# fusioninfer/fusioninfer

Hardware: AMD Instinct MI355X
Metric: goodput req/s (Qwen3-8B serving, closed-loop) (higher is better)
Workload: dtype bf16; 1 GPU; model=Qwen3-8B, global_batch=256, seq_len=1152, prompt_len=1024, gen_len=128, parallelism=dp1

## Files before the change

fusioninfer_amd/ops/__init__.py:

```python

from __future__ import annotations

import math
from typing import Optional

import torch

from fusioninfer_amd.ops import reference as ref

_C = None
_C_IMPORT_ERROR: Optional[BaseException] = None
try:
    import importlib

    _C = importlib.import_module("fusioninfer_amd.ops._C")
except Exception as e:
    _C_IMPORT_ERROR = e


def has_native() -> bool:
    return _C is not None


def _require_native():
# ... 148 lines not shown
        if (k_cache.dim() != 4 or k_cache.shape != v_cache.shape
                or k_cache.shape[1] != num_kv_heads or k_cache.shape[2] != 16
                or k_cache.shape[3] != head_dim):
            raise ValueError(
                "rope_qk_norm_cache_: caches must both be "
                f"[B, {num_kv_heads}, 16, {head_dim}], got "
                f"{tuple(k_cache.shape)} and {tuple(v_cache.shape)}")
        _C.rope_qk_norm_cache(
            q, k, v, q_weight, k_weight, cos_sin, positions, k_cache,
            v_cache, slot_mapping, num_q_heads, num_kv_heads, head_dim, eps,
            k_inv_scale, v_inv_scale,
        )
        return q
    rope_qk_norm_(q, k, positions, cos_sin, num_q_heads, num_kv_heads,
                  head_dim, q_weight, k_weight, eps)
    reshape_and_cache(k, v, k_cache, v_cache, slot_mapping,
                      k_inv_scale, v_inv_scale)
    return q


def gather_kv_blocks(k_cache, v_cache, block_ids) -> torch.Tensor:
    if k_cache.is_cuda:
        _require_native()
        n = int(block_ids.numel())
        staging = torch.empty(
            (2, n, *k_cache.shape[1:]), dtype=k_cache.dtype, device=k_cache.device
        )
        _C.gather_kv_blocks(staging, k_cache, v_cache, block_ids)
        return staging
    return ref.gather_kv_blocks(k_cache, v_cache, block_ids.long())


def scatter_kv_blocks(staging, k_cache, v_cache, block_ids):
    if k_cache.is_cuda:
        _require_native()
        _C.scatter_kv_blocks(staging, k_cache, v_cache, block_ids)
        return
    ref.scatter_kv_blocks(staging, k_cache, v_cache, block_ids.long())



DECODE_PARTITION_TOKENS = 512


def _check_attn_out(out: torch.Tensor, q: torch.Tensor) -> None:
    if (out.shape != q.shape or out.dtype != q.dtype
            or out.device != q.device or not out.is_contiguous()):
        raise ValueError(
            f"out must be a contiguous {tuple(q.shape)} {q.dtype} tensor on "
            f"{q.device}, got {tuple(out.shape)} {out.dtype} strides "
            f"{out.stride()} on {out.device}")


def paged_attention_decode(
    q: torch.Tensor,
    k_cache: torch.Tensor,
    v_cache: torch.Tensor,
    block_tables: torch.Tensor,
    seq_lens: torch.Tensor,
    scale: Optional[float] = None,
    out: Optional[torch.Tensor] = None,
) -> torch.Tensor:
    if scale is None:
        scale = 1.0 / math.sqrt(q.shape[-1])
    if out is not None:
        _check_attn_out(out, q)
    if q.is_cuda:
        _require_native()
        S, Hq, D = q.shape
        if out is None:
            out = torch.empty(q.shape, dtype=q.dtype, device=q.device)
        max_tokens = int(block_tables.shape[1]) * int(k_cache.shape[2])
        num_parts = max(
            (max_tokens + DECODE_PARTITION_TOKENS - 1) // DECODE_PARTITION_TOKENS,
            1,
        )
        ml_ws = acc_ws = None
        if num_parts > 1:
            ml_ws = torch.empty(
                (S, Hq, num_parts, 2), dtype=torch.float32, device=q.device
            )
            acc_ws = torch.empty(
                (S, Hq, num_parts, D), dtype=torch.float32, device=q.device
            )
        _C.paged_attention_decode(
            out, q, k_cache, v_cache, block_tables, seq_lens,
            ml_ws, acc_ws, num_parts, scale,
        )
        return out
    res = ref.paged_attention_decode(q, k_cache, v_cache, block_tables, seq_lens, scale)
    return res if out is None else out.copy_(res)


import os as _os

PREFILL_TILE_ROWS = (4 if _os.environ.get("FI_PF_NW", "8").startswith("4")
                     else 8) * 32


def prefill_tile_rows(seq_lens) -> int:
    if seq_lens and max(seq_lens) >= 4096:
        return 128
    return PREFILL_TILE_ROWS


def build_prefill_tiles(seq_lens, device=None, rows=None):
    rows = rows or PREFILL_TILE_ROWS
    tile_seq, tile_row0 = [], []
    for s, L in enumerate(seq_lens):
        for r0 in range(0, L, rows):
            tile_seq.append(s)
            tile_row0.append(r0)
    return (
        torch.tensor(tile_seq, dtype=torch.int32, device=device),
        torch.tensor(tile_row0, dtype=torch.int32, device=device),
    )


def prefill_attention(
    q: torch.Tensor,
    k: torch.Tensor,
    v: torch.Tensor,
    cu_seqlens: torch.Tensor,
    scale: Optional[float] = None,
    tile_seq: Optional[torch.Tensor] = None,
    tile_row0: Optional[torch.Tensor] = None,
    tile_rows: Optional[int] = None,
) -> torch.Tensor:
    if scale is None:
        scale = 1.0 / math.sqrt(q.shape[-1])
    if q.is_cuda:
        _require_native()
        if tile_seq is None:
            lens = (cu_seqlens[1:] - cu_seqlens[:-1]).tolist()
            tile_rows = tile_rows or prefill_tile_rows(lens)
            tile_seq, tile_row0 = build_prefill_tiles(
                lens, device=q.device, rows=tile_rows
            )
        out = torch.empty(q.shape, dtype=q.dtype, device=q.device)
        _C.prefill_attention(out, q, k, v, tile_seq, tile_row0, cu_seqlens,
# ... 274 lines not shown
```

fusioninfer_amd/ops/csrc/ops.hip:

```cpp

#include <torch/extension.h>

#include <c10/hip/HIPStream.h>
#include <hip/hip_runtime.h>

#include "common.h"

namespace fi {

template <bool FUSED_ADD, bool FP8_OUT>
void launch_rms_norm(void*, float*, const u16*, u16*, const u16*, float, int,
                     int, hipStream_t);
void launch_silu_and_mul(u16*, const u16*, int64_t, int, hipStream_t);
template <bool SILU_MUL>
void launch_row_quant_fp8(unsigned char*, float*, const u16*, int, int,
                          hipStream_t);
void launch_rope_qk_norm(u16*, u16*, int64_t, int64_t, const u16*, const u16*,
                         const float*, const int*, int, int, int, int, float,
                         hipStream_t);
void launch_reshape_and_cache(const u16*, const u16*, void*, void*,
                              const int*, int64_t, int64_t, int, int, int,
                              int, bool, float, float, hipStream_t);
void launch_rope_qk_norm_cache(u16*, const u16*, const u16*, int64_t, int64_t,
                               int64_t, const u16*, const u16*, const float*,
                               const int*, void*, void*, const int*, int, int,
                               int, int, float, bool, float, float,
                               hipStream_t);
template <bool GATHER>
void launch_kv_block_copy(u16*, u16*, u16*, const int*, int, int64_t,
                          hipStream_t);
void launch_paged_attn_decode(u16*, float*, float*, const u16*, const void*,
                              const void*, const int*, const int*, int,
                              int64_t, int, int, int, int, int, float, bool,
                              hipStream_t);
void launch_prefill_attn(u16*, const u16*, const void*, const void*,
                         const int*, const int*, const int*, const int*,
                         const int*, int, int, int64_t, int64_t, int64_t, int,
                         int, int, float, bool, int, hipStream_t);
void launch_moe_gemm(u16*, const u16*, const u16*, const int*, const int*,
                     const int*, int, int, int, int, bool, hipStream_t);
void launch_moe_gemm_fp8(u16*, const unsigned char*, const float*,
                         const unsigned char*, const float*, const int*,
                         const int*, const int*, int, int, int, int, bool,
                         hipStream_t);
void launch_moe_align(const int*, int*, int*, int*, int*, int, int, int,
                      int, int, int, hipStream_t);
void launch_moe_router_topk(const float*, float*, int*, int, int, int,
                            bool, hipStream_t);
void launch_moe_combine(u16*, const u16*, const int*, const float*, int, int,
                        int, hipStream_t);
void launch_lora_apply(u16*, u16*, const u16*, const int*, const u16*,
                       const u16*, const float*, int, int, int, int, int,
                       hipStream_t);
void launch_sample_tokens(int64_t*, const float*, const float*, const int*,
                          const float*, const float*, const int64_t*, int,
                          int, hipStream_t);
void launch_apply_penalties(float*, const int*, const int*, const float*, int,
                            int, int, hipStream_t);
void launch_penalty_counts_add(int*, const int*, const int64_t*, int, int,
                               int, hipStream_t);

}

namespace {

using fi::u16;

#define CHECK_BF16_CUDA(t)                                     \
  TORCH_CHECK((t).is_cuda(), #t " must be on GPU");            \
  TORCH_CHECK((t).scalar_type() == at::kBFloat16, #t " must be bf16")

u16* bf16_ptr(at::Tensor& t) { return reinterpret_cast<u16*>(t.data_ptr()); }
const u16* bf16_cptr(const at::Tensor& t) {
  return reinterpret_cast<const u16*>(t.data_ptr());
}

hipStream_t current_stream() {
  return c10::hip::getCurrentHIPStream().stream();
}

bool cache_is_fp8(const at::Tensor& t) {
  TORCH_CHECK(
      t.scalar_type() == at::kBFloat16 || t.scalar_type() == at::kFloat8_e4m3fn,
      "kv cache must be bf16 or float8_e4m3fn");
  return t.scalar_type() == at::kFloat8_e4m3fn;
}

// ... 183 lines not shown
    if (!w) return nullptr;
    CHECK_BF16_CUDA(*w);
    TORCH_CHECK(w->is_contiguous() && w->numel() == head_dim && aligned16(*w));
    return bf16_cptr(*w);
  };
  const u16* qw = weight_ptr(q_weight);
  const u16* kw = weight_ptr(k_weight);
  fi::launch_rope_qk_norm_cache(
      bf16_ptr(q), bf16_cptr(k), bf16_cptr(v), q.stride(0), k.stride(0),
      v.stride(0), qw, kw, cos_sin.data_ptr<float>(),
      positions.data_ptr<int>(), k_cache.data_ptr(), v_cache.data_ptr(),
      slot_mapping.data_ptr<int>(), static_cast<int>(tokens),
      static_cast<int>(num_q_heads), static_cast<int>(num_kv_heads),
      static_cast<int>(head_dim), static_cast<float>(eps), fp8,
      static_cast<float>(k_inv_scale), static_cast<float>(v_inv_scale),
      current_stream());
}

void gather_kv_blocks(at::Tensor staging, at::Tensor k_cache,
                      at::Tensor v_cache, at::Tensor block_ids) {
  TORCH_CHECK(staging.is_cuda() &&
              staging.scalar_type() == k_cache.scalar_type());
  TORCH_CHECK(block_ids.scalar_type() == at::kInt);
  const int n = block_ids.size(0);
  const int64_t block_elems = k_cache.size(1) * k_cache.size(2) *
      k_cache.size(3) * k_cache.element_size() / 2;
  fi::launch_kv_block_copy<true>(
      static_cast<fi::u16*>(staging.data_ptr()),
      static_cast<fi::u16*>(k_cache.data_ptr()),
      static_cast<fi::u16*>(v_cache.data_ptr()), block_ids.data_ptr<int>(), n,
      block_elems, current_stream());
}

void scatter_kv_blocks(at::Tensor staging, at::Tensor k_cache,
                       at::Tensor v_cache, at::Tensor block_ids) {
  TORCH_CHECK(staging.is_cuda() &&
              staging.scalar_type() == k_cache.scalar_type());
  TORCH_CHECK(block_ids.scalar_type() == at::kInt);
  const int n = block_ids.size(0);
  const int64_t block_elems = k_cache.size(1) * k_cache.size(2) *
      k_cache.size(3) * k_cache.element_size() / 2;
  fi::launch_kv_block_copy<false>(
      static_cast<fi::u16*>(staging.data_ptr()),
      static_cast<fi::u16*>(k_cache.data_ptr()),
      static_cast<fi::u16*>(v_cache.data_ptr()), block_ids.data_ptr<int>(), n,
      block_elems, current_stream());
}

void paged_attention_decode(at::Tensor out, at::Tensor q, at::Tensor k_cache,
                            at::Tensor v_cache, at::Tensor block_tables,
                            at::Tensor seq_lens,
                            c10::optional<at::Tensor> ml_ws,
                            c10::optional<at::Tensor> acc_ws,
                            int64_t num_parts, double scale) {
  CHECK_BF16_CUDA(out);
  CHECK_BF16_CUDA(q);
  const bool fp8 = cache_is_fp8(k_cache);
  TORCH_CHECK(block_tables.scalar_type() == at::kInt &&
              block_tables.is_contiguous());
  TORCH_CHECK(seq_lens.scalar_type() == at::kInt);
  TORCH_CHECK(q.dim() == 3);
  const int num_seqs = q.size(0);
  const int num_heads = q.size(1);
  const int head_dim = q.size(2);
  const int num_kv_heads = k_cache.size(1);
  TORCH_CHECK(k_cache.size(2) == 16, "cache block_size must be 16");
  TORCH_CHECK(q.stride(2) == 1 && q.stride(1) == head_dim);
  TORCH_CHECK(out.is_contiguous() && out.sizes() == q.sizes(),
              "out must be a contiguous [S, Hq, D] tensor");
  float* ml = nullptr;
  float* acc = nullptr;
  if (num_parts > 1) {
    TORCH_CHECK(ml_ws && acc_ws, "workspace required when num_parts > 1");
    ml = ml_ws->data_ptr<float>();
    acc = acc_ws->data_ptr<float>();
  }
  fi::launch_paged_attn_decode(
      bf16_ptr(out), ml, acc, bf16_cptr(q), k_cache.data_ptr(),
      v_cache.data_ptr(), block_tables.data_ptr<int>(),
      seq_lens.data_ptr<int>(), num_seqs, q.stride(0), block_tables.size(1),
      num_kv_heads, head_dim, num_heads / num_kv_heads,
      static_cast<int>(num_parts), static_cast<float>(scale), fp8,
      current_stream());
}

void prefill_attention(at::Tensor out, at::Tensor q, at::Tensor k,
                       at::Tensor v, at::Tensor tile_seq, at::Tensor tile_row0,
                       at::Tensor cu_seqlens, double scale,
                       int64_t tile_rows) {
  TORCH_CHECK(tile_rows == 128 || tile_rows == 256,
              "tile_rows must be 128 or 256");
  CHECK_BF16_CUDA(out);
  CHECK_BF16_CUDA(q);
  TORCH_CHECK(tile_seq.scalar_type() == at::kInt &&
              tile_row0.scalar_type() == at::kInt &&
              cu_seqlens.scalar_type() == at::kInt);
  TORCH_CHECK(q.dim() == 3 && k.dim() == 3 && v.dim() == 3);
  const int num_q_heads = q.size(1);
  const int head_dim = q.size(2);
  const int num_kv_heads = k.size(1);
  TORCH_CHECK(q.stride(2) == 1 && q.stride(1) == head_dim);
  TORCH_CHECK(k.stride(2) == 1 && k.stride(1) == head_dim);
  TORCH_CHECK(v.stride(2) == 1 && v.stride(1) == head_dim);
  fi::launch_prefill_attn(
      bf16_ptr(out), bf16_cptr(q), bf16_cptr(k), bf16_cptr(v),
      tile_seq.data_ptr<int>(), tile_row0.data_ptr<int>(),
      cu_seqlens.data_ptr<int>(), nullptr, nullptr, 0, tile_seq.size(0),
      q.stride(0), k.stride(0), v.stride(0), num_q_heads, num_kv_heads,
      head_dim, static_cast<float>(scale), false,
      static_cast<int>(tile_rows / 32), current_stream());
}

void prefill_attention_paged(at::Tensor out, at::Tensor q, at::Tensor k_cache,
                             at::Tensor v_cache, at::Tensor tile_seq,
                             at::Tensor tile_row0, at::Tensor cu_seqlens,
                             at::Tensor block_tables, at::Tensor seq_lens_k,
                             double scale, int64_t tile_rows) {
  TORCH_CHECK(tile_rows == 128 || tile_rows == 256,
              "tile_rows must be 128 or 256");
  CHECK_BF16_CUDA(out);
  CHECK_BF16_CUDA(q);
  const bool fp8 = cache_is_fp8(k_cache);
  TORCH_CHECK(tile_seq.scalar_type() == at::kInt &&
              tile_row0.scalar_type() == at::kInt &&
              cu_seqlens.scalar_type() == at::kInt &&
              block_tables.scalar_type() == at::kInt &&
              seq_lens_k.scalar_type() == at::kInt);
  TORCH_CHECK(block_tables.is_contiguous());
  TORCH_CHECK(q.dim() == 3);
  const int num_q_heads = q.size(1);
  const int head_dim = q.size(2);
  const int num_kv_heads = k_cache.size(1);
  TORCH_CHECK(k_cache.size(2) == 16, "cache block_size must be 16");
  TORCH_CHECK(q.stride(2) == 1 && q.stride(1) == head_dim);
  TORCH_CHECK(out.is_contiguous() && out.sizes() == q.sizes(),
              "out must be a contiguous [T, Hq, D] tensor");
// ... 227 lines not shown
      logits.data_ptr<float>(), counts.data_ptr<int>(),
      slot_ids.data_ptr<int>(), params.data_ptr<float>(),
      static_cast<int>(T), static_cast<int>(V),
      static_cast<int>(counts.size(0)), current_stream());
}

void penalty_counts_add(at::Tensor counts, at::Tensor slot_ids,
                        at::Tensor token_ids) {
  TORCH_CHECK(counts.is_cuda() && counts.scalar_type() == at::kInt &&
              counts.is_contiguous() && counts.dim() == 2 &&
              counts.size(0) >= 1 && counts.size(0) < (1LL << 31) &&
              counts.size(1) >= 1 && counts.size(1) < (1LL << 30),
              "penalty_counts_add: counts must be a contiguous [S >= 1, "
              "1 <= V < 2^30] int32 GPU tensor");
  const int64_t N = slot_ids.numel();
  TORCH_CHECK(N >= 1 && N < (1LL << 31) - 256,
              "penalty_counts_add: need 1 <= N < 2^31 - 256");
  TORCH_CHECK(slot_ids.is_cuda() && slot_ids.scalar_type() == at::kInt &&
              slot_ids.is_contiguous() && slot_ids.dim() == 1,
              "penalty_counts_add: bad slot_ids");
  TORCH_CHECK(token_ids.is_cuda() && token_ids.scalar_type() == at::kLong &&
              token_ids.is_contiguous() && token_ids.dim() == 1 &&
              token_ids.numel() == N,
              "penalty_counts_add: bad token_ids");
  fi::launch_penalty_counts_add(
      counts.data_ptr<int>(), slot_ids.data_ptr<int>(),
      token_ids.data_ptr<int64_t>(), static_cast<int>(N),
      static_cast<int>(counts.size(1)), static_cast<int>(counts.size(0)),
      current_stream());
}

}

PYBIND11_MODULE(TORCH_EXTENSION_NAME, m) {
  m.def("rms_norm", &rms_norm, "RMSNorm (bf16, fp32 accum)");
  m.def("fused_add_rms_norm", &fused_add_rms_norm,
        "in-place residual add + RMSNorm");
  m.def("silu_and_mul", &silu_and_mul, "fused SiLU-mul");
  m.def("rms_norm_fp8", &rms_norm_fp8, "RMSNorm with fused fp8 row quant");
  m.def("fused_add_rms_norm_fp8", &fused_add_rms_norm_fp8,
        "residual add + RMSNorm with fused fp8 row quant");
  m.def("silu_and_mul_fp8", &silu_and_mul_fp8,
        "fused SiLU-mul with fp8 row quant");
  m.def("quant_fp8_rows", &quant_fp8_rows, "per-row dynamic fp8 quant");
  m.def("rope_qk_norm", &rope_qk_norm,
        "fused per-head qk RMSNorm + NeoX RoPE (in-place)");
  m.def("reshape_and_cache", &reshape_and_cache, "scatter K/V into paged cache");
  m.def("rope_qk_norm_cache", &rope_qk_norm_cache,
        "fused qk RMSNorm + NeoX RoPE (q in place) + K/V paged-cache write");
  m.def("gather_kv_blocks", &gather_kv_blocks, "pack KV blocks for PD send");
  m.def("scatter_kv_blocks", &scatter_kv_blocks, "unpack KV blocks from PD recv");
  m.def("paged_attention_decode", &paged_attention_decode,
        "paged decode attention");
  m.def("prefill_attention", &prefill_attention, "varlen causal MFMA prefill");
  m.def("prefill_attention_paged", &prefill_attention_paged,
        "varlen causal MFMA prefill over the paged cache (context attention)");
  m.def("moe_gemm", &moe_gemm,
        "grouped MFMA GEMM over block-aligned expert segments "
        "(gate_up=true fuses the SwiGLU epilogue)");
  m.def("moe_gemm_fp8", &moe_gemm_fp8,
        "grouped fp8 (e4m3) MFMA GEMM with per-row/per-channel dequant "
        "epilogue (gate_up=true fuses SwiGLU)");
  m.def("moe_combine", &moe_combine,
        "weighted top-k combine of expert outputs (deterministic)");
  m.def("moe_align", &moe_align,
        "single-kernel block alignment of expert assignments "
        "(vLLM moe_align_block_size analog)");
  m.def("moe_router_topk", &moe_router_topk,
        "fused router tail: softmax + top-k + optional renormalize");
  m.def("lora_apply", &lora_apply,
        "batched multi-LoRA shrink + expand indexed by per-token slot ids "
        "(in-place on out)");
  m.def("sample_tokens", &sample_tokens,
        "fused temperature / top-k / top-p / min-p sampling with a "
        "counter-based (Philox4x32-10) draw, one workgroup per row");
  m.def("apply_penalties", &apply_penalties,
        "repetition / presence / frequency penalties from a per-slot token "
        "histogram (in-place on logits)");
  m.def("penalty_counts_add", &penalty_counts_add,
        "counts[slot_ids[i], token_ids[i]] += 1 (integer atomics)");
}
```

fusioninfer_amd/ops/csrc/paged_attention.hip:

```cpp

#include "common.h"

#include <type_traits>

namespace fi {

constexpr int kBlockSz = 16;
constexpr int kPartChunks = 32;
constexpr float kNegInf = -1e30f;
constexpr float kLog2e = 1.4426950408889634f;

typedef __attribute__((ext_vector_type(8))) short short8;
typedef __attribute__((ext_vector_type(4))) float floatx4;


template <typename CT_, int D, int G, int HS>
struct ScalarScores {
  using CT = CT_;
  static constexpr int G2 = G / HS, kTokLo = 4, kTokHi = 64;
  static constexpr int DPQ = D / 4;
  static constexpr int KQ4 = DPQ * sizeof(CT) / 16;
  static constexpr int EPG = 16 / sizeof(CT);
  struct KTile { uint4 v[KQ4]; };
  struct Q { const float (*heads)[D]; };

  static FI_DEV void init(Q& qs, const u16* q_row, float scale, int tid,
                          int nthreads, int, int hsplit) {
    __shared__ float q_lds[G][D];
    for (int e = tid; e < G * D; e += nthreads)
      q_lds[e / D][e % D] = bf16_to_f32(q_row[e]) * scale * kLog2e;
    __syncthreads();
    qs.heads = &q_lds[hsplit * G2];
  }

  static FI_DEV void load_k(const CT* k_block, int lane, KTile& k) {
    const CT* k_row = k_block + (lane / 4) * D + (lane % 4) * DPQ;
#pragma unroll
    for (int j8 = 0; j8 < KQ4; ++j8)
      k.v[j8] = reinterpret_cast<const uint4*>(k_row)[j8];
  }

  static FI_DEV void dot(const Q& qs, const KTile& k, int lane,
                         float (&s)[G2]) {
    const int quad = lane % 4;
#pragma unroll
    for (int g = 0; g < G2; ++g) s[g] = 0.f;
#pragma unroll
    for (int j8 = 0; j8 < KQ4; ++j8) {
      float kf8[EPG];
      if constexpr (sizeof(CT) == 1) {
        const u32 w[4] = {k.v[j8].x, k.v[j8].y, k.v[j8].z, k.v[j8].w};
#pragma unroll
        for (int i = 0; i < 4; ++i) unpack_fp8x4(w[i], &kf8[i * 4]);
      } else {
        const bf16x8 kv8 = __builtin_bit_cast(bf16x8, k.v[j8]);
#pragma unroll
        for (int j = 0; j < 8; ++j) kf8[j] = bf16_to_f32(kv8.h[j]);
      }
#pragma unroll
      for (int g = 0; g < G2; ++g) {
#pragma unroll
// ... 65 lines not shown
  using KTile = typename MfmaScoresBase<unsigned char, long long, D>::KTile;
  static constexpr int G2 = G / HS;
  struct Q {
    long long a[D / 32];
    float sc[G2];
  };

  static FI_DEV void init(Q& qs, const u16* q_row, float scale, int tid, int,
                          int lane, int hsplit) {
    __shared__ float qsc_lds[G];
    if (tid < G) {
      float mx = 1e-8f;
      for (int d = 0; d < D; ++d)
        mx = fmaxf(mx, fabsf(bf16_to_f32(q_row[tid * D + d])));
      qsc_lds[tid] = mx / 448.f;
    }
    __syncthreads();
    const int head = hsplit * G2 + ((lane & 15) % G2);
    const float inv_qs = 1.f / qsc_lds[head];
#pragma unroll
    for (int kk = 0; kk < D / 32; ++kk) {
      const int d0 = kk * 32 + (lane >> 4) * 8;
      float f[8];
#pragma unroll
      for (int e = 0; e < 8; ++e)
        f[e] = bf16_to_f32(q_row[head * D + d0 + e]) * inv_qs;
      u32 w[2];
      pack_fp8x8(f, w);
      qs.a[kk] = static_cast<long long>(
          (static_cast<unsigned long long>(w[1]) << 32) | w[0]);
    }
#pragma unroll
    for (int g = 0; g < G2; ++g)
      qs.sc[g] = qsc_lds[hsplit * G2 + g] * scale * kLog2e;
  }

  static FI_DEV void dot(const Q& qs, const KTile& k, int, float (&s)[G2]) {
    floatx4 c = {0.f, 0.f, 0.f, 0.f};
#pragma unroll
    for (int kk = 0; kk < D / 32; ++kk)
      c = __builtin_amdgcn_mfma_f32_16x16x32_fp8_fp8(qs.a[kk], k.v[kk], c, 0,
                                                     0, 0);
#pragma unroll
    for (int g = 0; g < G2; ++g) s[g] = c[g] * qs.sc[g];
  }
};

FI_DEV void store_out_pair(u16* o_row, int lane, float o0, float o1) {
  const u32 obits = static_cast<u32>(f32_to_bf16(o0)) |
                    (static_cast<u32>(f32_to_bf16(o1)) << 16);
  *reinterpret_cast<u32*>(o_row + 2 * lane) = obits;
}

template <template <int, int, int> class ScoresT, int D, int G, int kNWaves,
          int HS>
__global__ __launch_bounds__(kNWaves * kWaveSize) void paged_attn_decode_kernel(
    u16* __restrict__ out,
    float* __restrict__ ml_ws,
    float* __restrict__ acc_ws,
    const u16* __restrict__ q,
    const void* __restrict__ k_cache_p,
    const void* __restrict__ v_cache_p,
    const int* __restrict__ block_tables,
    const int* __restrict__ seq_lens,
    const int64_t q_stride, const int max_blocks, const int num_kv_heads,
    const float scale) {
  static_assert(HS <= G && G % HS == 0 && kNWaves % HS == 0);
  using Scores = ScoresT<D, G, HS>;
  using CT = typename Scores::CT;
  constexpr bool kFp8 = sizeof(CT) == 1;
  const CT* k_cache = static_cast<const CT*>(k_cache_p);
  const CT* v_cache = static_cast<const CT*>(v_cache_p);
  const int seq = blockIdx.x;
  const int kv_head = blockIdx.y;
  const int part = blockIdx.z;
  const int num_parts = gridDim.z;
  const int tid = threadIdx.x;
  const int wave = tid / kWaveSize;
  const int lane = tid % kWaveSize;
  constexpr int G2 = G / HS;
  constexpr int kCWaves = kNWaves / HS;
  const int hsplit = wave % HS;
  const int cwave = wave / HS;

  const int ctx = seq_lens[seq];
  const int num_chunks = (ctx + kBlockSz - 1) / kBlockSz;
  const int chunk_lo = part * kPartChunks;
  const int chunk_hi = min(num_chunks, chunk_lo + kPartChunks);
  const int num_heads = num_kv_heads * G;

  if (chunk_lo >= num_chunks) {
    if (tid < G) {
      const int h = kv_head * G + tid;
      float* ml = ml_ws + ((static_cast<int64_t>(seq) * num_heads + h) *
                               num_parts + part) * 2;
      ml[0] = kNegInf;
      ml[1] = 0.f;
    }
    return;
  }

  __shared__ float p_lds[kNWaves][kBlockSz][G2];
  __shared__ float merge_m[kNWaves][G2];
  __shared__ float merge_l[kNWaves][G2];
  __shared__ float merge_acc[kNWaves][G2][D];

  typename Scores::Q qs;
  Scores::init(qs, q + seq * q_stride + static_cast<int64_t>(kv_head) * G * D,
               scale, tid, kNWaves * kWaveSize, lane, hsplit);

  float m[G2], l[G2], acc[G2][2];
#pragma unroll
  for (int g = 0; g < G2; ++g) {
    m[g] = kNegInf;
    l[g] = 0.f;
    acc[g][0] = acc[g][1] = 0.f;
  }

  auto kv_base_of = [&](int chunk) -> int64_t {
    const int block_id = block_tables[seq * max_blocks + chunk];
    return ((static_cast<int64_t>(block_id) * num_kv_heads + kv_head) *
            kBlockSz) * D;
  };
  typename Scores::KTile kraw;
  int64_t kv_base = 0;
  if (chunk_lo + cwave < chunk_hi) {
    kv_base = kv_base_of(chunk_lo + cwave);
    Scores::load_k(k_cache + kv_base, lane, kraw);
  }

  constexpr int kTokLo = Scores::kTokLo, kTokHi = Scores::kTokHi;
  const int tok = (lane % kTokHi) / kTokLo;
  const bool parks_p = lane % kTokLo == 0 && lane < kTokHi;
  for (int chunk = chunk_lo + cwave; chunk < chunk_hi; chunk += kCWaves) {
    const int token_pos = chunk * kBlockSz + tok;
    const int64_t kv_base_cur = kv_base;

    float s[G2];
    Scores::dot(qs, kraw, lane, s);
    u32 vball[kBlockSz];
    const CT* v_rows = v_cache + kv_base_cur;
    if (lane < D / 2) {
#pragma unroll
      for (int t = 0; t < kBlockSz; ++t)
        vball[t] = kFp8
            ? static_cast<u32>(*reinterpret_cast<const u16*>(
                  v_rows + t * D + 2 * lane))
            : *reinterpret_cast<const u32*>(v_rows + t * D + 2 * lane);
    }
    if (chunk + kCWaves < chunk_hi) {
      kv_base = kv_base_of(chunk + kCWaves);
      Scores::load_k(k_cache + kv_base, lane, kraw);
    }
    __builtin_amdgcn_sched_barrier(0);
#pragma unroll
    for (int g = 0; g < G2; ++g) {
      if constexpr (kTokLo > 1) s[g] += __shfl_xor(s[g], 1, 64);
      if constexpr (kTokLo > 2) s[g] += __shfl_xor(s[g], 2, 64);
      if (token_pos >= ctx) s[g] = kNegInf;
    }

    float alpha[G2];
#pragma unroll
    for (int g = 0; g < G2; ++g) {
      float cm = s[g];
#pragma unroll
      for (int off = kTokLo; off < kTokHi; off <<= 1)
        cm = fmaxf(cm, __shfl_xor(cm, off, 64));
      const float m_new = fmaxf(m[g], cm);
      alpha[g] = __builtin_amdgcn_exp2f(m[g] - m_new);
      if (m[g] <= kNegInf && m_new <= kNegInf) alpha[g] = 0.f;
      m[g] = m_new;
    }

#pragma unroll
    for (int g = 0; g < G2; ++g) {
      float p = (s[g] <= kNegInf) ? 0.f
                : __builtin_amdgcn_exp2f(s[g] - m[g]);
      if (parks_p) p_lds[wave][tok][g] = p;
      float psum = p;
#pragma unroll
      for (int off = 1; off < kTokHi; off <<= 1)
        psum += __shfl_xor(psum, off, 64);
      l[g] = l[g] * alpha[g] + psum * (1.f / kTokLo);
    }

    __builtin_amdgcn_sched_barrier(0);
#pragma unroll
    for (int g = 0; g < G2; ++g) {
      acc[g][0] *= alpha[g];
      acc[g][1] *= alpha[g];
    }
    if (lane < D / 2) {
      for (int t = 0; t < kBlockSz; ++t) {
        float v0, v1;
        if (kFp8) {
          float vf[4];
          unpack_fp8x4(vball[t], vf);
          v0 = vf[0];
          v1 = vf[1];
        } else {
          v0 = bf16_to_f32(static_cast<u16>(vball[t] & 0xffff));
          v1 = bf16_to_f32(static_cast<u16>(vball[t] >> 16));
        }
#pragma unroll
        for (int g = 0; g < G2; ++g) {
          const float p = p_lds[wave][t][g];
          acc[g][0] = fmaf(p, v0, acc[g][0]);
          acc[g][1] = fmaf(p, v1, acc[g][1]);
        }
      }
    }
  }

  if (lane < G2) {
    merge_m[wave][lane] = m[lane];
    merge_l[wave][lane] = l[lane];
  }
  if (lane < D / 2) {
#pragma unroll
    for (int g = 0; g < G2; ++g) {
      merge_acc[wave][g][2 * lane] = acc[g][0];
      merge_acc[wave][g][2 * lane + 1] = acc[g][1];
    }
  }
  __syncthreads();

#pragma unroll
  for (int g = 0; g < G2; ++g) {
    if ((g % kCWaves) != cwave || lane >= D / 2) continue;
    float gm = kNegInf;
#pragma unroll
    for (int c = 0; c < kCWaves; ++c)
      gm = fmaxf(gm, merge_m[c * HS + hsplit][g]);
    float L = 0.f, o0 = 0.f, o1 = 0.f;
#pragma unroll
    for (int c = 0; c < kCWaves; ++c) {
      const int w = c * HS + hsplit;
      const float mw = merge_m[w][g];
      const float f = (mw <= kNegInf) ? 0.f
                      : __builtin_amdgcn_exp2f(mw - gm);
      L += merge_l[w][g] * f;
      o0 = fmaf(merge_acc[w][g][2 * lane], f, o0);
      o1 = fmaf(merge_acc[w][g][2 * lane + 1], f, o1);
    }
    const int h = kv_head * G + hsplit * G2 + g;
    if (num_parts == 1) {
      const float inv = 1.f / L;
      store_out_pair(out + (static_cast<int64_t>(seq) * num_heads + h) * D,
                     lane, o0 * inv, o1 * inv);
    } else {
      const int64_t slot = (static_cast<int64_t>(seq) * num_heads + h) *
                               gridDim.z + part;
      if (lane == 0) {
        ml_ws[slot * 2] = gm;
        ml_ws[slot * 2 + 1] = L;
      }
      float2* arow = reinterpret_cast<float2*>(acc_ws + slot * D);
      arow[lane] = make_float2(o0, o1);
    }
  }
}

template <int D>
__global__ __launch_bounds__(kWaveSize) void paged_attn_reduce_kernel(
    u16* __restrict__ out,
    const float* __restrict__ ml_ws,
    const float* __restrict__ acc_ws,
    const int num_parts) {
  const int seq = blockIdx.x;
  const int h = blockIdx.y;
  const int num_heads = gridDim.y;
  const int lane = threadIdx.x;
  if (lane >= D / 2) return;
  const int64_t base = (static_cast<int64_t>(seq) * num_heads + h) * num_parts;

  float gm = kNegInf;
  for (int p = 0; p < num_parts; ++p)
    gm = fmaxf(gm, ml_ws[(base + p) * 2]);
  float L = 0.f, o0 = 0.f, o1 = 0.f;
  for (int p = 0; p < num_parts; ++p) {
    const float mp = ml_ws[(base + p) * 2];
    if (mp <= kNegInf) continue;
    const float f = __builtin_amdgcn_exp2f(mp - gm);
    L += ml_ws[(base + p) * 2 + 1] * f;
    const float2 a =
        reinterpret_cast<const float2*>(acc_ws + (base + p) * D)[lane];
    o0 = fmaf(a.x, f, o0);
    o1 = fmaf(a.y, f, o1);
  }
  const float inv = 1.f / L;
  store_out_pair(out + (static_cast<int64_t>(seq) * num_heads + h) * D, lane,
                 o0 * inv, o1 * inv);
}

namespace {

struct DecodePlan {
  int nwaves, head_split;
  bool mfma_scores;
};

constexpr DecodePlan decode_plan(int group, bool wide, bool fp8, bool mfma) {
  return {wide ? 8 : 4, (group == 8 || (group == 4 && !wide)) ? 2 : 1,
          mfma && (!fp8 || group == 8)};
}

template <int D, int G, bool kWide, bool kFp8, bool kMfma, class... Args>
void launch_variant(dim3 grid, hipStream_t stream, Args... args) {
  constexpr DecodePlan p = decode_plan(G, kWide, kFp8, kMfma);
  constexpr int NW = p.nwaves, HS = p.head_split;
  auto launch = [&](auto kernel) {
    hipLaunchKernelGGL(kernel, grid, dim3(NW * kWaveSize), 0, stream, args...);
  };
  if constexpr (p.mfma_scores && kFp8)
    launch(paged_attn_decode_kernel<MfmaScoresFp8, D, G, NW, HS>);
  else if constexpr (p.mfma_scores)
    launch(paged_attn_decode_kernel<MfmaScoresBf16, D, G, NW, HS>);
  else if constexpr (kFp8)
    launch(paged_attn_decode_kernel<ScalarScoresFp8, D, G, NW, HS>);
  else
    launch(paged_attn_decode_kernel<ScalarScoresBf16, D, G, NW, HS>);
}

template <int D, int G, int kKey = 0, class... Args>
void launch_decode(int key, Args... args) {
  if constexpr (kKey < 8) {
    if (key != kKey) return launch_decode<D, G, kKey + 1>(key, args...);
    launch_variant<D, G, (kKey & 4) != 0, (kKey & 2) != 0, (kKey & 1) != 0>(
        args...);
  }
}

}

void launch_paged_attn_decode(u16* out, float* ml_ws, float* acc_ws,
                              const u16* q, const void* k_cache,
                              const void* v_cache, const int* block_tables,
                              const int* seq_lens, int num_seqs,
                              int64_t q_stride, int max_blocks,
                              int num_kv_heads, int head_dim, int group,
                              int num_parts, float scale, bool fp8,
                              hipStream_t stream) {
  const bool wide = num_seqs * num_kv_heads * num_parts < 256;
  static const bool mfma = [] {
    const char* e = getenv("FI_DECODE_MFMA");
    return !(e && e[0] == '0');
  }();
  const dim3 grid(num_seqs, num_kv_heads, num_parts);
  auto launch = [&](auto d, auto g) {
    constexpr int D = decltype(d)::value, G = decltype(g)::value;
    launch_decode<D, G>(wide << 2 | fp8 << 1 | mfma, grid, stream, out, ml_ws,
                        acc_ws, q, k_cache, v_cache, block_tables, seq_lens,
                        q_stride, max_blocks, num_kv_heads, scale);
    if (num_parts > 1) {
      dim3 rgrid(num_seqs, num_kv_heads * G), rblock(kWaveSize);
      hipLaunchKernelGGL((paged_attn_reduce_kernel<D>), rgrid, rblock, 0,
                         stream, out, ml_ws, acc_ws, num_parts);
    }
  };
  auto launch_group = [&](auto d) {
    switch (group) {
      case 1: return launch(d, std::integral_constant<int, 1>{});
      case 2: return launch(d, std::integral_constant<int, 2>{});
      case 4: return launch(d, std::integral_constant<int, 4>{});
      case 8: return launch(d, std::integral_constant<int, 8>{});
      default: abort();
    }
  };
  if (head_dim == 128) launch_group(std::integral_constant<int, 128>{});
  else if (head_dim == 64) launch_group(std::integral_constant<int, 64>{});
  else abort();
}

}
```

Before: 49.92 req/s.

## Add single-pass paged decode attention with in-LDS partition combine and table prefetch

Adds a single-pass decode attention path: when the grid (seqs x kv heads) is large enough and there are at most 4 partitions, one workgroup walks all partitions sequentially and combines them in shared memory. This drops the workspace allocations, the global ml/acc writes and the separate reduce kernel launch. Block-table entries are also prefetched into registers and read with readlane instead of per-chunk global loads. The cost is less parallelism per sequence, extra LDS use, and extra syncthreads between partitions.

```diff
diff --git a/fusioninfer_amd/ops/__init__.py b/fusioninfer_amd/ops/__init__.py
--- a/fusioninfer_amd/ops/__init__.py
+++ b/fusioninfer_amd/ops/__init__.py
@@ -224,6 +224,24 @@
             f"{out.stride()} on {out.device}")
 
 
+DECODE_SINGLE_PASS_MAX_PARTS = 4
+
+
+def decode_num_parts(table_blocks: int, block_size: int = 16) -> int:
+    max_tokens = int(table_blocks) * int(block_size)
+    return max(
+        (max_tokens + DECODE_PARTITION_TOKENS - 1) // DECODE_PARTITION_TOKENS, 1
+    )
+
+
+def decode_single_pass(num_seqs: int, num_kv_heads: int,
+                       table_blocks: int, fp8: bool = False) -> bool:
+    _require_native()
+    return bool(_C.decode_single_pass(
+        int(num_seqs), int(num_kv_heads), decode_num_parts(table_blocks),
+        bool(fp8)))
+
+
 def paged_attention_decode(
     q: torch.Tensor,
     k_cache: torch.Tensor,
@@ -232,6 +250,7 @@
     seq_lens: torch.Tensor,
     scale: Optional[float] = None,
     out: Optional[torch.Tensor] = None,
+    single_pass: Optional[bool] = None,
 ) -> torch.Tensor:
     if scale is None:
         scale = 1.0 / math.sqrt(q.shape[-1])
@@ -242,13 +261,18 @@
         S, Hq, D = q.shape
         if out is None:
             out = torch.empty(q.shape, dtype=q.dtype, device=q.device)
-        max_tokens = int(block_tables.shape[1]) * int(k_cache.shape[2])
-        num_parts = max(
-            (max_tokens + DECODE_PARTITION_TOKENS - 1) // DECODE_PARTITION_TOKENS,
-            1,
-        )
+        num_parts = decode_num_parts(block_tables.shape[1], k_cache.shape[2])
+        if single_pass is None:
+            single_pass = bool(_C.decode_single_pass(
+                S, int(k_cache.shape[1]), num_parts,
+                k_cache.dtype != torch.bfloat16))
+        elif single_pass and num_parts > DECODE_SINGLE_PASS_MAX_PARTS:
+            raise ValueError(
+                f"single_pass=True takes at most "
+                f"{DECODE_SINGLE_PASS_MAX_PARTS} partitions, the "
+                f"{int(block_tables.shape[1])}-block table has {num_parts}")
         ml_ws = acc_ws = None
-        if num_parts > 1:
+        if num_parts > 1 and not single_pass:
             ml_ws = torch.empty(
                 (S, Hq, num_parts, 2), dtype=torch.float32, device=q.device
             )
@@ -257,7 +281,7 @@
             )
         _C.paged_attention_decode(
             out, q, k_cache, v_cache, block_tables, seq_lens,
-            ml_ws, acc_ws, num_parts, scale,
+            ml_ws, acc_ws, num_parts, scale, bool(single_pass),
         )
         return out
     res = ref.paged_attention_decode(q, k_cache, v_cache, block_tables, seq_lens, scale)
diff --git a/fusioninfer_amd/ops/csrc/ops.hip b/fusioninfer_amd/ops/csrc/ops.hip
--- a/fusioninfer_amd/ops/csrc/ops.hip
+++ b/fusioninfer_amd/ops/csrc/ops.hip
@@ -32,7 +32,8 @@
 void launch_paged_attn_decode(u16*, float*, float*, const u16*, const void*,
                               const void*, const int*, const int*, int,
                               int64_t, int, int, int, int, int, float, bool,
-                              hipStream_t);
+                              bool, hipStream_t);
+bool decode_single_pass(int, int, int, bool);
 void launch_prefill_attn(u16*, const u16*, const void*, const void*,
                          const int*, const int*, const int*, const int*,
                          const int*, int, int, int64_t, int64_t, int64_t, int,
@@ -322,7 +323,8 @@
                             at::Tensor seq_lens,
                             c10::optional<at::Tensor> ml_ws,
                             c10::optional<at::Tensor> acc_ws,
-                            int64_t num_parts, double scale) {
+                            int64_t num_parts, double scale,
+                            bool single_pass) {
   CHECK_BF16_CUDA(out);
   CHECK_BF16_CUDA(q);
   const bool fp8 = cache_is_fp8(k_cache);
@@ -340,7 +342,9 @@
               "out must be a contiguous [S, Hq, D] tensor");
   float* ml = nullptr;
   float* acc = nullptr;
-  if (num_parts > 1) {
+  TORCH_CHECK(!single_pass || num_parts <= 4,
+              "the single pass takes tables of at most 4 partitions");
+  if (num_parts > 1 && !single_pass) {
     TORCH_CHECK(ml_ws && acc_ws, "workspace required when num_parts > 1");
     ml = ml_ws->data_ptr<float>();
     acc = acc_ws->data_ptr<float>();
@@ -351,7 +355,14 @@
       seq_lens.data_ptr<int>(), num_seqs, q.stride(0), block_tables.size(1),
       num_kv_heads, head_dim, num_heads / num_kv_heads,
       static_cast<int>(num_parts), static_cast<float>(scale), fp8,
-      current_stream());
+      single_pass, current_stream());
+}
+
+bool decode_single_pass(int64_t num_seqs, int64_t num_kv_heads,
+                        int64_t num_parts, bool fp8) {
+  return fi::decode_single_pass(static_cast<int>(num_seqs),
+                                static_cast<int>(num_kv_heads),
+                                static_cast<int>(num_parts), fp8);
 }
 
 void prefill_attention(at::Tensor out, at::Tensor q, at::Tensor k,
@@ -685,6 +696,9 @@
   m.def("scatter_kv_blocks", &scatter_kv_blocks, "unpack KV blocks from PD recv");
   m.def("paged_attention_decode", &paged_attention_decode,
         "paged decode attention");
+  m.def("decode_single_pass", &decode_single_pass,
+        "whether paged_attention_decode takes the single pass for "
+        "(num_seqs, num_kv_heads, num_parts, fp8 cache)");
   m.def("prefill_attention", &prefill_attention, "varlen causal MFMA prefill");
   m.def("prefill_attention_paged", &prefill_attention_paged,
         "varlen causal MFMA prefill over the paged cache (context attention)");
diff --git a/fusioninfer_amd/ops/csrc/paged_attention.hip b/fusioninfer_amd/ops/csrc/paged_attention.hip
--- a/fusioninfer_amd/ops/csrc/paged_attention.hip
+++ b/fusioninfer_amd/ops/csrc/paged_attention.hip
@@ -7,6 +7,11 @@
 
 constexpr int kBlockSz = 16;
 constexpr int kPartChunks = 32;
+constexpr int kMaxSinglePassParts = 4;
+#ifndef FI_DECODE_TABLE_PREFETCH
+#define FI_DECODE_TABLE_PREFETCH 1
+#endif
+constexpr bool kTablePrefetch = FI_DECODE_TABLE_PREFETCH != 0;
 constexpr float kNegInf = -1e30f;
 constexpr float kLog2e = 1.4426950408889634f;
 
@@ -178,8 +183,28 @@
   *reinterpret_cast<u32*>(o_row + 2 * lane) = obits;
 }
 
+template <class MlOf, class AccOf>
+FI_DEV void combine_partitions(u16* o_row, int lane, int num_parts,
+                               MlOf ml_of, AccOf acc_of) {
+  float gm = kNegInf;
+  for (int p = 0; p < num_parts; ++p)
+    gm = fmaxf(gm, ml_of(p)[0]);
+  float L = 0.f, o0 = 0.f, o1 = 0.f;
+  for (int p = 0; p < num_parts; ++p) {
+    const float mp = ml_of(p)[0];
+    if (mp <= kNegInf) continue;
+    const float f = __builtin_amdgcn_exp2f(mp - gm);
+    L += ml_of(p)[1] * f;
+    const float2 a = reinterpret_cast<const float2*>(acc_of(p))[lane];
+    o0 = fmaf(a.x, f, o0);
+    o1 = fmaf(a.y, f, o1);
+  }
+  const float inv = 1.f / L;
+  store_out_pair(o_row, lane, o0 * inv, o1 * inv);
+}
+
 template <template <int, int, int> class ScoresT, int D, int G, int kNWaves,
-          int HS>
+          int HS, bool kSinglePass>
 __global__ __launch_bounds__(kNWaves * kWaveSize) void paged_attn_decode_kernel(
     u16* __restrict__ out,
     float* __restrict__ ml_ws,
@@ -190,7 +215,7 @@
     const int* __restrict__ block_tables,
     const int* __restrict__ seq_lens,
     const int64_t q_stride, const int max_blocks, const int num_kv_heads,
-    const float scale) {
+    const int num_parts, const float scale) {
   static_assert(HS <= G && G % HS == 0 && kNWaves % HS == 0);
   using Scores = ScoresT<D, G, HS>;
   using CT = typename Scores::CT;
@@ -199,8 +224,6 @@
   const CT* v_cache = static_cast<const CT*>(v_cache_p);
   const int seq = blockIdx.x;
   const int kv_head = blockIdx.y;
-  const int part = blockIdx.z;
-  const int num_parts = gridDim.z;
   const int tid = threadIdx.x;
   const int wave = tid / kWaveSize;
   const int lane = tid % kWaveSize;
@@ -211,15 +234,19 @@
 
   const int ctx = seq_lens[seq];
   const int num_chunks = (ctx + kBlockSz - 1) / kBlockSz;
-  const int chunk_lo = part * kPartChunks;
-  const int chunk_hi = min(num_chunks, chunk_lo + kPartChunks);
   const int num_heads = num_kv_heads * G;
-
-  if (chunk_lo >= num_chunks) {
+  const int part_lo = kSinglePass ? 0 : blockIdx.z;
+  const int part_hi =
+      kSinglePass
+          ? max(min((num_chunks + kPartChunks - 1) / kPartChunks, num_parts), 1)
+          : part_lo + 1;
+  const int stream_hi = min(num_chunks, part_hi * kPartChunks);
+
+  if (!kSinglePass && part_lo * kPartChunks >= num_chunks) {
     if (tid < G) {
       const int h = kv_head * G + tid;
       float* ml = ml_ws + ((static_cast<int64_t>(seq) * num_heads + h) *
-                               num_parts + part) * 2;
+                               num_parts + part_lo) * 2;
       ml[0] = kNegInf;
       ml[1] = 0.f;
     }
@@ -230,160 +257,213 @@
   __shared__ float merge_m[kNWaves][G2];
   __shared__ float merge_l[kNWaves][G2];
   __shared__ float merge_acc[kNWaves][G2][D];
+  constexpr int kLdsParts = kSinglePass ? kMaxSinglePassParts : 1;
+  __shared__ float part_ml[kLdsParts][G][2];
+  __shared__ float part_acc[kLdsParts][G][D];
 
   typename Scores::Q qs;
   Scores::init(qs, q + seq * q_stride + static_cast<int64_t>(kv_head) * G * D,
                scale, tid, kNWaves * kWaveSize, lane, hsplit);
 
-  float m[G2], l[G2], acc[G2][2];
-#pragma unroll
-  for (int g = 0; g < G2; ++g) {
-    m[g] = kNegInf;
-    l[g] = 0.f;
-    acc[g][0] = acc[g][1] = 0.f;
-  }
-
+  constexpr int kTabRegs =
+      !kTablePrefetch ? 0
+      : kSinglePass   ? kMaxSinglePassParts * kPartChunks / kWaveSize
+                      : 1;
+  const int* table_row = block_tables + seq * max_blocks;
+  const int tab_lo = part_lo * kPartChunks;
+  int tab[kTabRegs > 0 ? kTabRegs : 1];
+#pragma unroll
+  for (int r = 0; r < kTabRegs; ++r) {
+    const int e = tab_lo + r * kWaveSize + lane;
+    tab[r] = e < stream_hi ? table_row[e] : 0;
+  }
   auto kv_base_of = [&](int chunk) -> int64_t {
-    const int block_id = block_tables[seq * max_blocks + chunk];
+    int block_id;
+    if constexpr (kTablePrefetch) {
+      const int i = __builtin_amdgcn_readfirstlane(chunk - tab_lo);
+      block_id = __builtin_amdgcn_readlane(tab[0], i & (kWaveSize - 1));
+#pragma unroll
+      for (int r = 1; r < kTabRegs; ++r)
+        if (i >= r * kWaveSize)
+          block_id = __builtin_amdgcn_readlane(tab[r], i & (kWaveSize - 1));
+    } else {
+      block_id = table_row[chunk];
+    }
     return ((static_cast<int64_t>(block_id) * num_kv_heads + kv_head) *
             kBlockSz) * D;
   };
+
+  static_assert(kPartChunks % kCWaves == 0);
   typename Scores::KTile kraw;
   int64_t kv_base = 0;
-  if (chunk_lo + cwave < chunk_hi) {
-    kv_base = kv_base_of(chunk_lo + cwave);
+  if (tab_lo + cwave < stream_hi) {
+    kv_base = kv_base_of(tab_lo + cwave);
     Scores::load_k(k_cache + kv_base, lane, kraw);
   }
 
   constexpr int kTokLo = Scores::kTokLo, kTokHi = Scores::kTokHi;
   const int tok = (lane % kTokHi) / kTokLo;
   const bool parks_p = lane % kTokLo == 0 && lane < kTokHi;
-  for (int chunk = chunk_lo + cwave; chunk < chunk_hi; chunk += kCWaves) {
-    const int token_pos = chunk * kBlockSz + tok;
-    const int64_t kv_base_cur = kv_base;
-
-    float s[G2];
-    Scores::dot(qs, kraw, lane, s);
-    u32 vball[kBlockSz];
-    const CT* v_rows = v_cache + kv_base_cur;
+
+  int part = part_lo;
+  do {
+    const int chunk_lo = part * kPartChunks;
+    const int chunk_hi = min(num_chunks, chunk_lo + kPartChunks);
+    float m[G2], l[G2], acc[G2][2];
+#pragma unroll
+    for (int g = 0; g < G2; ++g) {
+      m[g] = kNegInf;
+      l[g] = 0.f;
+      acc[g][0] = acc[g][1] = 0.f;
+    }
+
+    for (int chunk = chunk_lo + cwave; chunk < chunk_hi; chunk += kCWaves) {
+      const int token_pos = chunk * kBlockSz + tok;
+      const int64_t kv_base_cur = kv_base;
+
+      float s[G2];
+      Scores::dot(qs, kraw, lane, s);
+      u32 vball[kBlockSz];
+      const CT* v_rows = v_cache + kv_base_cur;
+      if (lane < D / 2) {
+#pragma unroll
+        for (int t = 0; t < kBlockSz; ++t)
+          vball[t] = kFp8
+              ? static_cast<u32>(*reinterpret_cast<const u16*>(
+                    v_rows + t * D + 2 * lane))
+              : *reinterpret_cast<const u32*>(v_rows + t * D + 2 * lane);
+      }
+      if (chunk + kCWaves < stream_hi) {
+        kv_base = kv_base_of(chunk + kCWaves);
+        Scores::load_k(k_cache + kv_base, lane, kraw);
+      }
+      __builtin_amdgcn_sched_barrier(0);
+#pragma unroll
+      for (int g = 0; g < G2; ++g) {
+        if constexpr (kTokLo > 1) s[g] += __shfl_xor(s[g], 1, 64);
+        if constexpr (kTokLo > 2) s[g] += __shfl_xor(s[g], 2, 64);
+        if (token_pos >= ctx) s[g] = kNegInf;
+      }
+
+      float alpha[G2];
+#pragma unroll
+      for (int g = 0; g < G2; ++g) {
+        float cm = s[g];
+#pragma unroll
+        for (int off = kTokLo; off < kTokHi; off <<= 1)
+          cm = fmaxf(cm, __shfl_xor(cm, off, 64));
+        const float m_new = fmaxf(m[g], cm);
+        alpha[g] = __builtin_amdgcn_exp2f(m[g] - m_new);
+        if (m[g] <= kNegInf && m_new <= kNegInf) alpha[g] = 0.f;
+        m[g] = m_new;
+      }
+
+#pragma unroll
+      for (int g = 0; g < G2; ++g) {
+        float p = (s[g] <= kNegInf) ? 0.f
+                  : __builtin_amdgcn_exp2f(s[g] - m[g]);
+        if (parks_p) p_lds[wave][tok][g] = p;
+        float psum = p;
+#pragma unroll
+        for (int off = 1; off < kTokHi; off <<= 1)
+          psum += __shfl_xor(psum, off, 64);
+        l[g] = l[g] * alpha[g] + psum * (1.f / kTokLo);
+      }
+
+      __builtin_amdgcn_sched_barrier(0);
+#pragma unroll
+      for (int g = 0; g < G2; ++g) {
+        acc[g][0] *= alpha[g];
+        acc[g][1] *= alpha[g];
+      }
+      if (lane < D / 2) {
+        for (int t = 0; t < kBlockSz; ++t) {
+          float v0, v1;
+          if (kFp8) {
+            float vf[4];
+            unpack_fp8x4(vball[t], vf);
+            v0 = vf[0];
+            v1 = vf[1];
+          } else {
+            v0 = bf16_to_f32(static_cast<u16>(vball[t] & 0xffff));
+            v1 = bf16_to_f32(static_cast<u16>(vball[t] >> 16));
+          }
+#pragma unroll
+          for (int g = 0; g < G2; ++g) {
+            const float p = p_lds[wave][t][g];
+            acc[g][0] = fmaf(p, v0, acc[g][0]);
+            acc[g][1] = fmaf(p, v1, acc[g][1]);
+          }
+        }
+      }
+    }
+
+    if (kSinglePass && part > part_lo) __syncthreads();
+    if (lane < G2) {
+      merge_m[wave][lane] = m[lane];
+      merge_l[wave][lane] = l[lane];
+    }
     if (lane < D / 2) {
 #pragma unroll
-      for (int t = 0; t < kBlockSz; ++t)
-        vball[t] = kFp8
-            ? static_cast<u32>(*reinterpret_cast<const u16*>(
-                  v_rows + t * D + 2 * lane))
-            : *reinterpret_cast<const u32*>(v_rows + t * D + 2 * lane);
-    }
-    if (chunk + kCWaves < chunk_hi) {
-      kv_base = kv_base_of(chunk + kCWaves);
-      Scores::load_k(k_cache + kv_base, lane, kraw);
-    }
-    __builtin_amdgcn_sched_barrier(0);
+      for (int g = 0; g < G2; ++g) {
+        merge_acc[wave][g][2 * lane] = acc[g][0];
+        merge_acc[wave][g][2 * lane + 1] = acc[g][1];
+      }
+    }
+    __syncthreads();
+
 #pragma unroll
     for (int g = 0; g < G2; ++g) {
-      if constexpr (kTokLo > 1) s[g] += __shfl_xor(s[g], 1, 64);
-      if constexpr (kTokLo > 2) s[g] += __shfl_xor(s[g], 2, 64);
-      if (token_pos >= ctx) s[g] = kNegInf;
-    }
-
-    float alpha[G2];
+      if ((g % kCWaves) != cwave || lane >= D / 2) continue;
+      float gm = kNegInf;
+#pragma unroll
+      for (int c = 0; c < kCWaves; ++c)
+        gm = fmaxf(gm, merge_m[c * HS + hsplit][g]);
+      float L = 0.f, o0 = 0.f, o1 = 0.f;
+#pragma unroll
+      for (int c = 0; c < kCWaves; ++c) {
+        const int w = c * HS + hsplit;
+        const float mw = merge_m[w][g];
+        const float f = (mw <= kNegInf) ? 0.f
+                        : __builtin_amdgcn_exp2f(mw - gm);
+        L += merge_l[w][g] * f;
+        o0 = fmaf(merge_acc[w][g][2 * lane], f, o0);
+        o1 = fmaf(merge_acc[w][g][2 * lane + 1], f, o1);
+      }
+      const int hb = hsplit * G2 + g;
+      const int h = kv_head * G + hb;
+      if constexpr (kSinglePass) {
+        part_ml[part][hb][0] = gm;
+        part_ml[part][hb][1] = L;
+        reinterpret_cast<float2*>(part_acc[part][hb])[lane] =
+            make_float2(o0, o1);
+      } else if (num_parts == 1) {
+        const float inv = 1.f / L;
+        store_out_pair(out + (static_cast<int64_t>(seq) * num_heads + h) * D,
+                       lane, o0 * inv, o1 * inv);
+      } else {
+        const int64_t slot = (static_cast<int64_t>(seq) * num_heads + h) *
+                                 num_parts + part;
+        if (lane == 0) {
+          ml_ws[slot * 2] = gm;
+          ml_ws[slot * 2 + 1] = L;
+        }
+        float2* arow = reinterpret_cast<float2*>(acc_ws + slot * D);
+        arow[lane] = make_float2(o0, o1);
+      }
+    }
+  } while (kSinglePass && ++part < part_hi);
+
+  if constexpr (kSinglePass) {
 #pragma unroll
     for (int g = 0; g < G2; ++g) {
-      float cm = s[g];
-#pragma unroll
-      for (int off = kTokLo; off < kTokHi; off <<= 1)
-        cm = fmaxf(cm, __shfl_xor(cm, off, 64));
-      const float m_new = fmaxf(m[g], cm);
-      alpha[g] = __builtin_amdgcn_exp2f(m[g] - m_new);
-      if (m[g] <= kNegInf && m_new <= kNegInf) alpha[g] = 0.f;
-      m[g] = m_new;
-    }
-
-#pragma unroll
-    for (int g = 0; g < G2; ++g) {
-      float p = (s[g] <= kNegInf) ? 0.f
-                : __builtin_amdgcn_exp2f(s[g] - m[g]);
-      if (parks_p) p_lds[wave][tok][g] = p;
-      float psum = p;
-#pragma unroll
-      for (int off = 1; off < kTokHi; off <<= 1)
-        psum += __shfl_xor(psum, off, 64);
-      l[g] = l[g] * alpha[g] + psum * (1.f / kTokLo);
-    }
-
-    __builtin_amdgcn_sched_barrier(0);
-#pragma unroll
-    for (int g = 0; g < G2; ++g) {
-      acc[g][0] *= alpha[g];
-      acc[g][1] *= alpha[g];
-    }
-    if (lane < D / 2) {
-      for (int t = 0; t < kBlockSz; ++t) {
-        float v0, v1;
-        if (kFp8) {
-          float vf[4];
-          unpack_fp8x4(vball[t], vf);
-          v0 = vf[0];
-          v1 = vf[1];
-        } else {
-          v0 = bf16_to_f32(static_cast<u16>(vball[t] & 0xffff));
-          v1 = bf16_to_f32(static_cast<u16>(vball[t] >> 16));
-        }
-#pragma unroll
-        for (int g = 0; g < G2; ++g) {
-          const float p = p_lds[wave][t][g];
-          acc[g][0] = fmaf(p, v0, acc[g][0]);
-          acc[g][1] = fmaf(p, v1, acc[g][1]);
-        }
-      }
-    }
-  }
-
-  if (lane < G2) {
-    merge_m[wave][lane] = m[lane];
-    merge_l[wave][lane] = l[lane];
-  }
-  if (lane < D / 2) {
-#pragma unroll
-    for (int g = 0; g < G2; ++g) {
-      merge_acc[wave][g][2 * lane] = acc[g][0];
-      merge_acc[wave][g][2 * lane + 1] = acc[g][1];
-    }
-  }
-  __syncthreads();
-
-#pragma unroll
-  for (int g = 0; g < G2; ++g) {
-    if ((g % kCWaves) != cwave || lane >= D / 2) continue;
-    float gm = kNegInf;
-#pragma unroll
-    for (int c = 0; c < kCWaves; ++c)
-      gm = fmaxf(gm, merge_m[c * HS + hsplit][g]);
-    float L = 0.f, o0 = 0.f, o1 = 0.f;
-#pragma unroll
-    for (int c = 0; c < kCWaves; ++c) {
-      const int w = c * HS + hsplit;
-      const float mw = merge_m[w][g];
-      const float f = (mw <= kNegInf) ? 0.f
-                      : __builtin_amdgcn_exp2f(mw - gm);
-      L += merge_l[w][g] * f;
-      o0 = fmaf(merge_acc[w][g][2 * lane], f, o0);
-      o1 = fmaf(merge_acc[w][g][2 * lane + 1], f, o1);
-    }
-    const int h = kv_head * G + hsplit * G2 + g;
-    if (num_parts == 1) {
-      const float inv = 1.f / L;
-      store_out_pair(out + (static_cast<int64_t>(seq) * num_heads + h) * D,
-                     lane, o0 * inv, o1 * inv);
-    } else {
-      const int64_t slot = (static_cast<int64_t>(seq) * num_heads + h) *
-                               gridDim.z + part;
-      if (lane == 0) {
-        ml_ws[slot * 2] = gm;
-        ml_ws[slot * 2 + 1] = L;
-      }
-      float2* arow = reinterpret_cast<float2*>(acc_ws + slot * D);
-      arow[lane] = make_float2(o0, o1);
+      if ((g % kCWaves) != cwave || lane >= D / 2) continue;
+      const int hb = hsplit * G2 + g;
+      const int h = kv_head * G + hb;
+      combine_partitions(
+          out + (static_cast<int64_t>(seq) * num_heads + h) * D, lane, part_hi,
+          [&](int p) { return part_ml[p][hb]; },
+          [&](int p) { return part_acc[p][hb]; });
     }
   }
 }
@@ -400,24 +480,10 @@
   const int lane = threadIdx.x;
   if (lane >= D / 2) return;
   const int64_t base = (static_cast<int64_t>(seq) * num_heads + h) * num_parts;
-
-  float gm = kNegInf;
-  for (int p = 0; p < num_parts; ++p)
-    gm = fmaxf(gm, ml_ws[(base + p) * 2]);
-  float L = 0.f, o0 = 0.f, o1 = 0.f;
-  for (int p = 0; p < num_parts; ++p) {
-    const float mp = ml_ws[(base + p) * 2];
-    if (mp <= kNegInf) continue;
-    const float f = __builtin_amdgcn_exp2f(mp - gm);
-    L += ml_ws[(base + p) * 2 + 1] * f;
-    const float2 a =
-        reinterpret_cast<const float2*>(acc_ws + (base + p) * D)[lane];
-    o0 = fmaf(a.x, f, o0);
-    o1 = fmaf(a.y, f, o1);
-  }
-  const float inv = 1.f / L;
-  store_out_pair(out + (static_cast<int64_t>(seq) * num_heads + h) * D, lane,
-                 o0 * inv, o1 * inv);
+  combine_partitions(
+      out + (static_cast<int64_t>(seq) * num_heads + h) * D, lane, num_parts,
+      [&](int p) { return ml_ws + (base + p) * 2; },
+      [&](int p) { return acc_ws + (base + p) * D; });
 }
 
 namespace {
@@ -432,7 +498,23 @@
           mfma && (!fp8 || group == 8)};
 }
 
-template <int D, int G, bool kWide, bool kFp8, bool kMfma, class... Args>
+constexpr int kSinglePassMinGrid = 768;
+constexpr bool single_pass_plan(int num_seqs, int num_kv_heads, int num_parts,
+                                bool fp8, bool mfma) {
+  return num_seqs * num_kv_heads >= kSinglePassMinGrid && num_parts > 1 &&
+         num_parts <= kMaxSinglePassParts && mfma && !fp8;
+}
+
+bool mfma_enabled() {
+  static const bool mfma = [] {
+    const char* e = getenv("FI_DECODE_MFMA");
+    return !(e && e[0] == '0');
+  }();
+  return mfma;
+}
+
+template <int D, int G, bool kSingle, bool kWide, bool kFp8, bool kMfma,
+          class... Args>
 void launch_variant(dim3 grid, hipStream_t stream, Args... args) {
   constexpr DecodePlan p = decode_plan(G, kWide, kFp8, kMfma);
   constexpr int NW = p.nwaves, HS = p.head_split;
@@ -440,24 +522,34 @@
     hipLaunchKernelGGL(kernel, grid, dim3(NW * kWaveSize), 0, stream, args...);
   };
   if constexpr (p.mfma_scores && kFp8)
-    launch(paged_attn_decode_kernel<MfmaScoresFp8, D, G, NW, HS>);
+    launch(paged_attn_decode_kernel<MfmaScoresFp8, D, G, NW, HS, kSingle>);
   else if constexpr (p.mfma_scores)
-    launch(paged_attn_decode_kernel<MfmaScoresBf16, D, G, NW, HS>);
+    launch(paged_attn_decode_kernel<MfmaScoresBf16, D, G, NW, HS, kSingle>);
   else if constexpr (kFp8)
-    launch(paged_attn_decode_kernel<ScalarScoresFp8, D, G, NW, HS>);
+    launch(paged_attn_decode_kernel<ScalarScoresFp8, D, G, NW, HS, kSingle>);
   else
-    launch(paged_attn_decode_kernel<ScalarScoresBf16, D, G, NW, HS>);
+    launch(paged_attn_decode_kernel<ScalarScoresBf16, D, G, NW, HS, kSingle>);
 }
 
 template <int D, int G, int kKey = 0, class... Args>
 void launch_decode(int key, Args... args) {
-  if constexpr (kKey < 8) {
+  if constexpr (kKey < 16) {
     if (key != kKey) return launch_decode<D, G, kKey + 1>(key, args...);
-    launch_variant<D, G, (kKey & 4) != 0, (kKey & 2) != 0, (kKey & 1) != 0>(
-        args...);
-  }
-}
-
+    launch_variant<D, G, (kKey & 8) != 0, (kKey & 4) != 0, (kKey & 2) != 0,
+                   (kKey & 1) != 0>(args...);
+  }
+}
+
+}
+
+bool decode_single_pass(int num_seqs, int num_kv_heads, int num_parts,
+                        bool fp8) {
+  static const bool enabled = [] {
+    const char* e = getenv("FI_DECODE_SINGLE_PASS");
+    return !(e && e[0] == '0');
+  }();
+  return enabled && single_pass_plan(num_seqs, num_kv_heads, num_parts, fp8,
+                                     mfma_enabled());
 }
 
 void launch_paged_attn_decode(u16* out, float* ml_ws, float* acc_ws,
@@ -467,19 +559,18 @@
                               int64_t q_stride, int max_blocks,
                               int num_kv_heads, int head_dim, int group,
                               int num_parts, float scale, bool fp8,
-                              hipStream_t stream) {
+                              bool single_pass, hipStream_t stream) {
+  if (single_pass && num_parts > kMaxSinglePassParts) abort();
   const bool wide = num_seqs * num_kv_heads * num_parts < 256;
-  static const bool mfma = [] {
-    const char* e = getenv("FI_DECODE_MFMA");
-    return !(e && e[0] == '0');
-  }();
-  const dim3 grid(num_seqs, num_kv_heads, num_parts);
+  const bool mfma = mfma_enabled();
+  const dim3 grid(num_seqs, num_kv_heads, single_pass ? 1 : num_parts);
   auto launch = [&](auto d, auto g) {
     constexpr int D = decltype(d)::value, G = decltype(g)::value;
-    launch_decode<D, G>(wide << 2 | fp8 << 1 | mfma, grid, stream, out, ml_ws,
-                        acc_ws, q, k_cache, v_cache, block_tables, seq_lens,
-                        q_stride, max_blocks, num_kv_heads, scale);
-    if (num_parts > 1) {
+    launch_decode<D, G>(single_pass << 3 | wide << 2 | fp8 << 1 | mfma, grid,
+                        stream, out, ml_ws, acc_ws, q, k_cache, v_cache,
+                        block_tables, seq_lens, q_stride, max_blocks,
+                        num_kv_heads, num_parts, scale);
+    if (num_parts > 1 && !single_pass) {
       dim3 rgrid(num_seqs, num_kv_heads * G), rblock(kWaveSize);
       hipLaunchKernelGGL((paged_attn_reduce_kernel<D>), rgrid, rblock, 0,
                          stream, out, ml_ws, acc_ws, num_parts);
```

Result: slower. 49.04 req/s (-1.8%).
